# pypr/pysph

Hardware: AMD Instinct MI355X
Metric: particle-updates/sec (nnps.update + AccelerationEval.compute), WCSPH 3D, fp64 (higher is better)
Workload: dtype f64

## Files before the change

pysph_amd/csrc/sph_eval.hip:

```cpp
#include "sph_internal.h"
#include "sph_kernels.h"
#include "sph_pair.h"

#include <cfloat>
#include <cmath>
#include <type_traits>

#ifndef SPH_KERNEL_UNIT
#define SPH_KERNEL_UNIT 0
#endif
#define SPH_PRIMARY_UNIT (SPH_KERNEL_UNIT == 0)

#if SPH_PRIMARY_UNIT

struct EosArgs {
    int kind;
    double par[SPH_MAX_PAR];
    double *rho, *p, *cs;
    size_t start, stop;
    double *q[SPH_PROP_COUNT];
    uint32_t *tflag;
};

__device__ inline void jacobi_eigen3(double A[3][3], double V[3][3], double d[3])
// ... 304 lines not shown
#pragma unroll
            for (int q = 0; q < MAX_AUX / 2; q++) pc[2 + q] = make_double2(v[2 * q], v[2 * q + 1]);
            np = a.nr / 2;
        }
        emit_pieces(a, i, pc, np);
    } else {
        a.posh[a.off + i] = ph;
        double *dst = a.aux + (a.off + i) * (size_t)a.na;
#pragma unroll
        for (int k = 0; k < MAX_AUX; k++) if (k < a.na) dst[k] = v[k];
    }
}

struct PackMArgs {
    const uint32_t *perm;
    const uint8_t *slot;
    size_t n, off;
    const double *prop[9][SPH_MAX_ARRAYS];
    int vh;
    uint32_t cls;
    double *rec;
    float4 *fpos;
    int f32, lds_np;
    double gmin[3];
    double hr;
    uint32_t *rho_flag;
};

template <bool F32, bool VH>
__global__ __launch_bounds__(256) void k_pack_merged(PackMArgs a)
{
    const size_t i = (size_t)blockIdx.x * blockDim.x + threadIdx.x;
    if (i >= a.n) return;
    const uint32_t o = a.perm[i], sl = a.slot[i];
    double v[8];
#pragma unroll
    for (int k = 0; k < 8; k++) {
        const double *p = kernarg_read<const double *>(__builtin_offsetof(PackMArgs, prop) + ((size_t)k * SPH_MAX_ARRAYS + sl) * sizeof(double *));
        v[k] = p[o];
    }
    const double rho = v[6];
    const double q = rho != 0.0 ? v[7] * (1.0 / (rho * rho)) : 0.0;
    const double srho = ((a.cls >> sl) & 1u) ? -rho : rho;
    if (!(rho > 0.0) && fabs(v[0]) < SPH_PARKED_MIN) atomicOr(a.rho_flag, 1u);
    double hp = 0.0;
    if (VH) hp = kernarg_read<const double *>(__builtin_offsetof(PackMArgs, prop) + ((size_t)8 * SPH_MAX_ARRAYS + sl) * sizeof(double *))[o];
    a.fpos[i] = make_float4((float)(v[0] - a.gmin[0]), (float)(v[1] - a.gmin[1]), (float)(v[2] - a.gmin[2]),
                            VH ? (float)(a.hr * hp) : (float)a.hr);
    double2 pc[PACK_MAXP];
#pragma unroll
    for (int k = 0; k < PACK_MAXP; k++) pc[k] = make_double2(0.0, 0.0);
    int np;
    if (VH && F32) {
        pc[0] = __builtin_bit_cast(double2, make_float4((float)(v[0] - a.gmin[0]), (float)(v[1] - a.gmin[1]), (float)(v[2] - a.gmin[2]), (float)hp));
        pc[1] = __builtin_bit_cast(double2, make_float4((float)v[3], (float)v[4], (float)v[5], (float)srho));
        np = 2;
    } else if (VH) {
        pc[0] = make_double2(v[0], v[1]); pc[1] = make_double2(v[2], hp);
        pc[2] = make_double2(v[3], v[4]); pc[3] = make_double2(v[5], srho);
        np = 4;
    } else if (F32) {
        pc[0] = __builtin_bit_cast(double2, make_float4((float)(v[0] - a.gmin[0]), (float)(v[1] - a.gmin[1]), (float)(v[2] - a.gmin[2]), (float)v[3]));
        pc[1] = __builtin_bit_cast(double2, make_float4((float)v[4], (float)v[5], (float)srho, (float)q));
        np = 2;
    } else {
        pc[0] = make_double2(v[0], v[1]); pc[1] = make_double2(v[2], v[3]);
        pc[2] = make_double2(v[4], v[5]); pc[3] = make_double2(srho, q);
        np = 4;
    }
    emit_pieces(a, i, pc, np);
}

template <class T> struct FamWCSPH_T {
    typedef T Real;
    static constexpr uint32_t CF0 = F_CONT | F_MOM | F_XSPH;
#ifndef SPH_WCSPH_MINB
#define SPH_WCSPH_MINB 4
#endif
    static constexpr int MINB = SPH_WCSPH_MINB;
    static constexpr int NA = 8;
    static constexpr int NR = 12;
    struct Params {
        T c0, alpha, beta, gx, gy, gz, eps;
        double *arho, *au, *av, *aw, *ax, *ay, *az, *dt_cfl, *dt_force;
    };
    struct Dest {
        T u, v, w, rho, p, cs, tmpi;
        T arho, au, av, aw, ax, ay, az, dt_cfl;
    };
    template <class A> static __device__ __forceinline__ void load(Dest &D, const T *a, const A &, uint32_t)
    {
        D.u = a[0]; D.v = a[1]; D.w = a[2]; D.rho = a[4]; D.tmpi = a[5]; D.cs = a[6]; D.p = a[7];
        D.arho = D.au = D.av = D.aw = D.ax = D.ay = D.az = T(0.0);
        D.dt_cfl = T(-1.0);
    }
    static constexpr bool PRED = true;
    template <int KK, bool UH, class A>
    static __device__ __forceinline__ void pair(Dest &D, const real4<T> &pi, const real4<T> &pj, T r2,
                                                const T (&s)[NA], uint32_t fl, const A &a, bool pass = true)
    {
        PairGeomT<T> g;
        constexpr bool MRG = SPH_MERGED_RSQ && sizeof(T) == 8 && !SphKernel<KK>::CUTOFF;
        T tt_m = T(0.0);
        if constexpr (MRG) {
            if (fl & F_MOM) tt_m = pair_geom_mom<KK, UH>(g, pi, pj, r2, T(0.5) * (D.rho + s[4]), a);
            else pair_geom<KK, UH>(g, pi, pj, r2, a);
        } else {
            pair_geom<KK, UH>(g, pi, pj, r2, a);
        }
        const T tg = pair_gradfac<KK, UH>(g);
        const T vij0 = D.u - s[0], vij1 = D.v - s[1], vij2 = D.w - s[2];
        const T vdotx = vij0 * g.xij[0] + vij1 * g.xij[1] + vij2 * g.xij[2];
        const T mj = pass ? s[3] : T(0.0);
        if (fl & F_CONT) D.arho = fma(mj * tg, vdotx, D.arho);
        if (fl & (F_MOM | F_XSPH)) {
            const T rhoij = T(0.5) * (D.rho + s[4]);
            T rhoij1;
            T wij = T(0.0);
            if (fl & (F_XSPH | F_TENSILE)) wij = pair_w<KK, UH>(g);
            if (fl & F_MOM) {
                const T re = r2 + g.eps;
                const T tt = MRG ? tt_m : fast_rcp(re * rhoij);
                const T inv_re = rhoij * tt;
                rhoij1 = re * tt;
                const T hv = g.hij * vdotx;
                const T muij = raw_min(hv, T(0.0)) * inv_re;
                const T cij = T(0.5) * (D.cs + s[6]);
                const T piij = (a.p.beta * muij - a.p.alpha * cij) * muij * rhoij1;
                const T dtv = fabs(hv * (g.rinv * g.rinv));
                D.dt_cfl = raw_max(D.dt_cfl, (r2 > T(1e-12) && pass) ? dtv : T(-1.0));
                const T tmpj = s[5];
                T tmp = D.tmpi + tmpj;
                if (fl & F_TENSILE) {
                    const T qd = (a.k.deltap * g.hij) * g.h1;
                    const T wdp = SphKernel<KK>::w(qd, g.dim) * g.fac;
                    T fij = wij * fast_rcp(wdp);
                    fij = fij * fij;
                    fij = fij * fij;
                    const T Ri = D.p > 0 ? T(0.01) * D.tmpi : T(0.2) * fabs(D.tmpi);
                    const T Rj = s[7] > 0 ? T(0.01) * tmpj : T(0.2) * fabs(tmpj);
                    tmp = (D.tmpi + tmpj) + (Ri + Rj) * fij;
                }
                const T ft = -mj * (tmp + piij) * tg;
                D.au = fma(ft, g.xij[0], D.au);
                D.av = fma(ft, g.xij[1], D.av);
                D.aw = fma(ft, g.xij[2], D.aw);
            } else {
                rhoij1 = fast_rcp(rhoij);
            }
            if (fl & F_XSPH) {
                const T tmp = -a.p.eps * mj * wij * rhoij1;
                D.ax = fma(tmp, vij0, D.ax);
                D.ay = fma(tmp, vij1, D.ay);
                D.az = fma(tmp, vij2, D.az);
            }
        }
    }
    template <class A> static __device__ __forceinline__ void finish(Dest &D, const A &a, uint32_t o)
    {
        if (a.dflags & F_CONT) a.p.arho[o] = D.arho;
        if (a.dflags & F_MOM) {
            T au = D.au + a.p.gx, av = D.av + a.p.gy, aw = D.aw + a.p.gz;
            a.p.au[o] = au; a.p.av[o] = av; a.p.aw[o] = aw;
            a.p.dt_cfl[o] = D.dt_cfl < T(0.0) ? T(0.0) : D.dt_cfl + a.p.c0;
            a.p.dt_force[o] = au * au + av * av + aw * aw;
        }
        if (a.dflags & F_XSPH) {
            a.p.ax[o] = D.ax + D.u; a.p.ay[o] = D.ay + D.v; a.p.az[o] = D.az + D.w;
        }
    }
};
typedef FamWCSPH_T<double> FamWCSPH;

template <class T, bool UM = false> struct FamWCSPHE_T : FamWCSPH_T<T> {
    static constexpr bool EOSF = true;
    static constexpr bool UMASS = UM;
    static constexpr int NR = 8;
    struct Raw {
        typename std::conditional<sizeof(T) == 8, double2, float4>::type q[sizeof(T) == 8 ? 4 : 2];
    };
    template <class A> static __device__ __forceinline__ void load_raw(const A &a, uint32_t jg, Raw &r)
    {
        if constexpr (sizeof(T) == 8) {
            const double2 *p = reinterpret_cast<const double2 *>(a.rec) + (unsigned long long)jg * 4;
            r.q[0] = p[0]; r.q[1] = p[1]; r.q[2] = p[2]; r.q[3] = p[3];
        } else {
            const float4 *p = reinterpret_cast<const float4 *>(a.rec) + (unsigned long long)jg * 2;
            r.q[0] = p[0]; r.q[1] = p[1];
        }
    }
    template <class A> static __device__ __forceinline__ void decode(const A &a, const Raw &r, uint32_t fl, T mu, real4<T> &pj, T (&s)[8],
                                                                     int gk = 3)
    {
        T rho;
        if constexpr (sizeof(T) == 8) {
            pj.x = r.q[0].x; pj.y = r.q[0].y; pj.z = r.q[1].x; pj.w = 0.0;
            s[0] = r.q[1].y; s[1] = r.q[2].x; s[2] = r.q[2].y; s[3] = r.q[3].y; rho = r.q[3].x;
        } else {
            pj.x = r.q[0].x; pj.y = r.q[0].y; pj.z = r.q[0].z; pj.w = 0.f;
            s[0] = r.q[0].w; s[1] = r.q[1].x; s[2] = r.q[1].y; s[3] = r.q[1].w; rho = r.q[1].z;
        }
        s[4] = rho;
        s[5] = s[6] = s[7] = T(0.0);
        if constexpr (UM) {
            const T q = s[3];
            s[3] = mu;
            if (fl & F_MOM) {
                const T ratio = rho * (T)a.e_rho01;
                s[5] = q;
                s[6] = (T)a.e_c0 * tait_cs_power(ratio, gk);
            }
        } else
        if (fl & F_MOM) {
            const T ratio = rho * (T)a.e_rho01;
            T r7, r3;
            tait_powers(ratio, gk, r7, r3);
            const T p = (T)a.e_p0 + (T)a.e_B * (r7 - T(1.0));
            s[5] = rho != T(0.0) ? p * fast_rcp(rho * rho) : T(0.0);
            s[6] = (T)a.e_c0 * r3;
            s[7] = p;
        }
    }
    template <class A> static __device__ __forceinline__ void load_fused(const A &a, uint32_t jg, uint32_t fl, T mu, real4<T> &pj, T (&s)[8])
    {
        Raw r;
        load_raw(a, jg, r);
        decode(a, r, fl, mu, pj, s);
    }
};

template <class T, bool UM = false> struct FamWCSPHEG_T : FamWCSPHE_T<T, UM> {
    typedef FamWCSPHE_T<T, UM> Base;
    template <class A> static __device__ __forceinline__ void load_fused(const A &a, uint32_t jg, uint32_t fl, T mu, real4<T> &pj, T (&s)[8])
    {
        typename Base::Raw r;
        Base::load_raw(a, jg, r);
        Base::decode(a, r, fl, mu, pj, s, a.e_gk);
    }
};

template <class T> struct FamWCSPHV_T : FamWCSPH_T<T> {
    static constexpr bool EOSF = true;
    static constexpr int NR = 8;
    template <class A> static __device__ __forceinline__ void load_fused(const A &a, uint32_t jg, uint32_t fl, T mu, real4<T> &pj, T (&s)[8])
    {
        T rho;
        if constexpr (sizeof(T) == 8) {
            const double2 *p = reinterpret_cast<const double2 *>(a.rec) + (unsigned long long)jg * 4;
            const double2 q0 = p[0], q1 = p[1], q2 = p[2], q3 = p[3];
            pj.x = q0.x; pj.y = q0.y; pj.z = q1.x; pj.w = q1.y;
            s[0] = q2.x; s[1] = q2.y; s[2] = q3.x; rho = q3.y;
        } else {
            const float4 *p = reinterpret_cast<const float4 *>(a.rec) + (unsigned long long)jg * 2;
            const float4 q0 = p[0], q1 = p[1];
            pj.x = q0.x; pj.y = q0.y; pj.z = q0.z; pj.w = q0.w;
            s[0] = q1.x; s[1] = q1.y; s[2] = q1.z; rho = q1.w;
        }
        s[3] = mu;
        s[4] = rho;
        s[5] = s[6] = s[7] = T(0.0);
        if (fl & F_MOM) {
            const T ratio = rho * (T)a.e_rho01;
            T r7, r3;
            tait_powers(ratio, 3, r7, r3);
            const T p = (T)a.e_p0 + (T)a.e_B * (r7 - T(1.0));
            s[5] = rho != T(0.0) ? p * fast_rcp(rho * rho) : T(0.0);
            s[6] = (T)a.e_c0 * r3;
            s[7] = p;
        }
    }
};

#define WCSPHM_CT(f00, f01, f10, f11) ((uint32_t)(f00) | ((uint32_t)(f01) << 4) | ((uint32_t)(f10) << 8) | ((uint32_t)(f11) << 12))
template <class T> struct FamWCSPHM_T : FamWCSPHE_T<T, true> {
    typedef FamWCSPHE_T<T, true> Base;
    typedef typename Base::Raw Raw;
    static constexpr bool MERGED = true;
    static constexpr uint32_t CF0 = WCSPHM_CT(F_CONT | F_MOM | F_XSPH, F_CONT | F_MOM, F_CONT, 0);
    struct Params {
        T c0, alpha, beta, gx, gy, gz, eps;
        double mu1;
        uint32_t rng[SPH_MAX_ARRAYS][2];
        double *out[SPH_MAX_ARRAYS][9];
    };
    static __device__ __forceinline__ size_t rng_offset(uint32_t slot) { return __builtin_offsetof(Params, rng) + (size_t)slot * 8; }
    struct Dest : Base::Dest { bool dc; };
    template <class A> static __device__ __forceinline__ void load(Dest &D, const T *a, const A &A_, uint32_t o, uint32_t)
    {
        Base::load(D, a, A_, o);
        D.dc = a[3] < T(0.0);
    }
    template <class A> static __device__ __forceinline__ void decode(const A &a, const Raw &r, uint32_t, T mu, real4<T> &pj, T (&s)[8])
    {
        T rho, q;
        if constexpr (sizeof(T) == 8) {
            pj.x = r.q[0].x; pj.y = r.q[0].y; pj.z = r.q[1].x; pj.w = 0.0;
            s[0] = r.q[1].y; s[1] = r.q[2].x; s[2] = r.q[2].y; q = r.q[3].y; rho = r.q[3].x;
        } else {
            pj.x = r.q[0].x; pj.y = r.q[0].y; pj.z = r.q[0].z; pj.w = 0.f;
            s[0] = r.q[0].w; s[1] = r.q[1].x; s[2] = r.q[1].y; q = r.q[1].w; rho = r.q[1].z;
        }
        const bool c1 = rho < T(0.0);
        s[3] = c1 ? -(T)a.p.mu1 : mu;
        rho = fabs(rho);
        s[4] = rho;
        const T ratio = rho * (T)a.e_rho01;
        s[5] = q;
        s[6] = (T)a.e_c0 * tait_cs_power(ratio, 3);
        s[7] = T(0.0);
    }
    template <class A> static __device__ __forceinline__ void load_fused(const A &a, uint32_t jg, uint32_t fl, T mu, real4<T> &pj, T (&s)[8])
    {
        Raw r;
        Base::load_raw(a, jg, r);
        decode(a, r, fl, mu, pj, s);
    }
    static __device__ __forceinline__ bool acts(uint32_t ct, uint32_t bit, bool dc, bool sc)
    {
        const bool c00 = ct & bit, c01 = (ct >> 4) & bit, c10 = (ct >> 8) & bit, c11 = (ct >> 12) & bit;
        return dc ? (sc ? c11 : c10) : (sc ? c01 : c00);
    }
    template <int KK, bool UH, class A>
    static __device__ __forceinline__ void pair(Dest &D, const real4<T> &pi, const real4<T> &pj, T r2,
                                                const T (&s)[8], uint32_t ct, const A &a, bool pass = true)
    {
        PairGeomT<T> g;
        constexpr bool MRG = SPH_MERGED_RSQ && sizeof(T) == 8 && !SphKernel<KK>::CUTOFF;
        T tt_m = T(0.0);
        if constexpr (MRG) tt_m = pair_geom_mom<KK, UH>(g, pi, pj, r2, T(0.5) * (D.rho + s[4]), a);
        else pair_geom<KK, UH>(g, pi, pj, r2, a);
        const T tg = pair_gradfac<KK, UH>(g);
        const T vij0 = D.u - s[0], vij1 = D.v - s[1], vij2 = D.w - s[2];
        const T vdotx = vij0 * g.xij[0] + vij1 * g.xij[1] + vij2 * g.xij[2];
        const bool sc = s[3] < T(0.0);
        const T m = fabs(s[3]);
        const bool on_c = pass && acts(ct, F_CONT, D.dc, sc), on_m = pass && acts(ct, F_MOM, D.dc, sc),
                   on_x = pass && acts(ct, F_XSPH, D.dc, sc);
        D.arho = fma((on_c ? m : T(0.0)) * tg, vdotx, D.arho);
        const T rhoij = T(0.5) * (D.rho + s[4]);
        const T wij = pair_w<KK, UH>(g);
        const T re = r2 + g.eps;
        const T tt = MRG ? tt_m : fast_rcp(re * rhoij);
        const T inv_re = rhoij * tt;
        const T rhoij1 = re * tt;
        const T hv = g.hij * vdotx;
        const T muij = raw_min(hv, T(0.0)) * inv_re;
        const T cij = T(0.5) * (D.cs + s[6]);
        const T piij = (a.p.beta * muij - a.p.alpha * cij) * muij * rhoij1;
        const T dtv = fabs(hv * (g.rinv * g.rinv));
        D.dt_cfl = raw_max(D.dt_cfl, (r2 > T(1e-12) && on_m) ? dtv : T(-1.0));
        const T ft = -(on_m ? m : T(0.0)) * ((D.tmpi + s[5]) + piij) * tg;
        D.au = fma(ft, g.xij[0], D.au);
        D.av = fma(ft, g.xij[1], D.av);
        D.aw = fma(ft, g.xij[2], D.aw);
        const T tmp = -a.p.eps * (on_x ? m : T(0.0)) * wij * rhoij1;
        D.ax = fma(tmp, vij0, D.ax);
        D.ay = fma(tmp, vij1, D.ay);
        D.az = fma(tmp, vij2, D.az);
    }
    template <class A> static __device__ __forceinline__ void finish(Dest &D, const A &a, uint32_t o, uint32_t slot)
// ... 1342 lines not shown
                for (auto &pc : c->pack_cache)
                    if (pc.epoch == c->pack_epoch && (pc.fam != fam || pc.sig != sig)) keep = false;
            if (!keep)
                for (auto &pc : c->pack_cache) pc.epoch = 0;
            auto pack_once = [&](int id, size_t off, uint32_t fl, bool dest_only) -> int {
                PackCache &pc = c->pack_cache[id];
                const bool hit = share && pc.epoch == c->pack_epoch && pc.fam == fam && pc.sig == sig;
                if (phase != 2 || repack) SPH_TRY(pack_array(c, id, off, pl, fam, fl, dest_only, !hit, 0));
                if (phase != 1 && c->arr[id].g_n > 0) SPH_TRY(pack_array(c, id, off, pl, fam, fl, dest_only, !hit, 1));
                pc.epoch = share ? c->pack_epoch : 0; pc.fam = fam; pc.sig = sig;
                return SPH_OK;
            };
            for (int j = 0; j < nsrcs; j++) SPH_TRY(pack_once(srcs[j], off_of[j], srcs[j] == dst ? dflags : sflags[j], false));
            if (!dest_is_src) SPH_TRY(pack_once(dst, d_off, dflags, true));
        }

        int nl_mode = 0;
        if (c->nl_reuse && !c->row_lds && c->pair_variant == 6 && nsrcs == 1 && g->nl_mode && !c->ablate && !any_ghosts && phase == 0) {
            const size_t n_wt = (size_t)4 * div_up(D.n, 256);
            if (g->nl_mode == 1) {
                SPH_TRY(c->nlbuf.reserve(n_wt * NLW * sizeof(uint32_t)));
                c->nl.valid = true; c->nl.epoch = c->nnps_epoch; c->nl.dst = dst; c->nl.src = srcs[0];
                c->nl.start = start; c->nl.stop = stop; c->nl.nd = D.n;
                nl_mode = 1;
            } else if (g->nl_mode == 2 && c->nl.valid && c->nl.epoch == c->nnps_epoch && c->nl.dst == dst && c->nl.src == srcs[0] &&
                       c->nl.nd == D.n && c->nl.start <= start && c->nl.stop >= stop && c->nlbuf.bytes >= n_wt * NLW * sizeof(uint32_t)) {
                nl_mode = 2;
            }
        } else if (g->nl_mode != 2) {
            c->nl.valid = c->nl.valid && !(g->nl_mode == 1);
        }

        if (phase == 1 && !c->split_pair) continue;
        ScopedTimer tm(c, T_PAIR);
        ScopedTimer tmf(c, T_PAIR_FAM + fam);
        if (phase == 2) c->timers[T_N_PHASE2].count++;
        if (eosf || tvff || eosv) c->timers[T_N_EOSF].count++;
        if (umass || tvff || elu || eosv) c->timers[T_N_UMASS].count++;
        if (nl_mode == 1) c->timers[T_N_NLKEEP].count++;
        if (nl_mode == 2) c->timers[T_N_NLREUSE].count++;
        {
            int nseg = nsrcs;
            for (int j = 0; j < nsrcs; j++) nseg += c->arr[srcs[j]].g_n > 0 && phase != 1;
            if (nseg > SPH_MAX_ARRAYS) { sph_set_error("too many source segments (%d arrays with ghost segments)", nsrcs); return SPH_ERR_UNSUPPORTED; }
        }
        auto common = [&](auto &a) {
            fill_common(c, a, K, t);
            a.nsrc = 0;
            for (int j = 0; j < nsrcs; j++) {
                const DevArray &S = c->arr[srcs[j]];
                a.src[a.nsrc++] = {S.cell_start.as<uint32_t>(), (uint32_t)off_of[j], sflags[j], S.fine_start.as<uint32_t>(), S.m_value, 0u};
            }
            for (int j = 0; j < nsrcs && phase != 1; j++) {
                const DevArray &S = c->arr[srcs[j]];
                if (S.g_n == 0) continue;
                a.src[a.nsrc++] = {S.g_cell_start.as<uint32_t>(), (uint32_t)(off_of[j] + S.n_binned), sflags[j],
                                   S.g_fine_start.as<uint32_t>(), S.m_value, 1u};
            }
            a.face_mode = c->split_pair ? phase : 0;
            a.d_off = (uint32_t)d_off; a.nd = (uint32_t)D.n_binned;
            a.d_mu = D.m_value;
            a.d_keys = D.keys_sorted.as<uint32_t>(); a.d_fkeys = D.fkeys_sorted.as<uint32_t>(); a.d_perm = D.perm.as<uint32_t>();
            set_tile_order(c, a, D);
            a.d_start = (uint32_t)start; a.d_stop = (uint32_t)stop; a.dflags = dflags;
            a.nl = nullptr; a.nl_mode = nl_mode;
            if (nl_mode) a.nl = c->nlbuf.as<uint32_t>();
            if (start == 0 && stop == D.n_real && D.n_binned == D.n && !any_ghosts) use_dest_list(c, a, D);
            if (eosf || eosv) {
                a.e_rho01 = 1.0 / g->eos_par[0]; a.e_c0 = g->eos_par[1];
                a.e_B = g->eos_par[0] * g->eos_par[1] * g->eos_par[1] / g->eos_par[2];
        a.e_gk = tait_gk(g->eos_par[2]);
                a.e_p0 = g->eos_par[3];
            }
            if (tvff) { a.e_p0 = g->eos_par[0]; a.e_rho01 = 1.0 / g->eos_par[1]; a.e_B = g->eos_par[2]; }
        };
        auto run_wcsph = [&](auto tag) -> int {
            typedef decltype(tag) F;
            PairArgs<F> a;
            memset(&a, 0, sizeof a);
            common(a);
            const sph_equation *me = eq_of[SPH_EQ_MOMENTUM], *xe = eq_of[SPH_EQ_XSPH];
            if (me) { a.p.c0 = me->par[0]; a.p.alpha = me->par[1]; a.p.beta = me->par[2]; a.p.gx = me->par[3]; a.p.gy = me->par[4]; a.p.gz = me->par[5]; }
            if (xe) a.p.eps = xe->par[0];
            if (dflags & F_CONT) { SPH_TRY(ensure_out(c, dst, {SPH_ARHO})); a.p.arho = D.prop[SPH_ARHO]; }
            if (dflags & F_MOM) {
                SPH_TRY(ensure_out(c, dst, {SPH_AU, SPH_AV, SPH_AW, SPH_DT_CFL, SPH_DT_FORCE}));
                a.p.au = D.prop[SPH_AU]; a.p.av = D.prop[SPH_AV]; a.p.aw = D.prop[SPH_AW];
                a.p.dt_cfl = D.prop[SPH_DT_CFL]; a.p.dt_force = D.prop[SPH_DT_FORCE];
            }
            if (dflags & F_XSPH) {
                SPH_TRY(ensure_out(c, dst, {SPH_AX, SPH_AY, SPH_AZ}));
                a.p.ax = D.prop[SPH_AX]; a.p.ay = D.prop[SPH_AY]; a.p.az = D.prop[SPH_AZ];
            }
            if constexpr (std::is_same<F, FamWCSPHV_T<typename F::Real>>::value) return launch_pair_fused<F, false>(c, K->kind, a);
            else if constexpr (fam_eosf<F>::value) return launch_pair_fused<F>(c, K->kind, a);
            else return launch_pair<F>(c, K->kind, a);
        };
        auto run_density = [&](auto tag) -> int {
            typedef decltype(tag) F;
            PairArgs<F> a;
            memset(&a, 0, sizeof a);
            common(a);
            SPH_TRY(ensure_out(c, dst, {SPH_RHO}));
            a.p.rho = D.prop[SPH_RHO];
            if (dflags & F_TVFSD) { SPH_TRY(ensure_out(c, dst, {SPH_VOL})); a.p.V = D.prop[SPH_VOL]; }
            if ((dflags & F_SD) && (dflags & F_TVFSD)) { sph_set_error("both SummationDensity flavours on one destination"); return SPH_ERR_UNSUPPORTED; }
            return launch_pair<F>(c, K->kind, a);
        };
        auto run_vgrad = [&](auto tag) -> int {
            typedef decltype(tag) F;
            PairArgs<F> a;
            memset(&a, 0, sizeof a);
            common(a);
            static const int vp[9] = {SPH_V00, SPH_V01, SPH_V02, SPH_V10, SPH_V11, SPH_V12, SPH_V20, SPH_V21, SPH_V22};
            if ((dflags & F_VG2) && (dflags & F_VG3)) { sph_set_error("both VelocityGradient2D and 3D on one destination"); return SPH_ERR_UNSUPPORTED; }
            for (int k = 0; k < 9; k++) {
                const bool used = (dflags & F_VG3) || (k == 0 || k == 1 || k == 3 || k == 4);
                if (used) { SPH_TRY(sph_array_ensure_prop(c, dst, vp[k])); a.p.v[k] = D.prop[vp[k]]; }
            }
            return launch_pair<F>(c, K->kind, a);
        };
        auto run_elastic = [&](auto tag) -> int {
            typedef decltype(tag) F;
            PairArgs<F> a;
            memset(&a, 0, sizeof a);
            common(a);
            const sph_equation *se = eq_of[SPH_EQ_MOMENTUM_WITH_STRESS], *ae = eq_of[SPH_EQ_MONAGHAN_ART_VISCOSITY],
                               *xe = eq_of[SPH_EQ_XSPH];
            if (se) { a.p.wdeltap = se->par[0]; a.p.n = se->par[1]; }
            a.p.tension = nullptr;
            if (elu && c->tension_flag && nsrcs == 1 && c->arr[srcs[0]].tflag_valid && c->arr[srcs[0]].tflag.ptr) {
                a.p.tension = c->arr[srcs[0]].tflag.as<uint32_t>();
                c->timers[T_N_TFLAG].count++;
            }
            if (ae) { a.p.alpha = ae->par[0]; a.p.beta = ae->par[1]; }
            if (xe) a.p.eps = xe->par[0];
            if (dflags & F_ECONT) { SPH_TRY(ensure_out(c, dst, {SPH_ARHO})); a.p.arho = D.prop[SPH_ARHO]; }
            if (dflags & (F_ESTRESS | F_EAV)) {
                SPH_TRY(ensure_out(c, dst, {SPH_AU, SPH_AV, SPH_AW}));
                a.p.au = D.prop[SPH_AU]; a.p.av = D.prop[SPH_AV]; a.p.aw = D.prop[SPH_AW];
            }
            if (dflags & F_EXSPH) {
                SPH_TRY(ensure_out(c, dst, {SPH_AX, SPH_AY, SPH_AZ}));
                a.p.ax = D.prop[SPH_AX]; a.p.ay = D.prop[SPH_AY]; a.p.az = D.prop[SPH_AZ];
            }
            if constexpr (fam_eosf<F>::value) return launch_pair_fused<F>(c, K->kind, a);
            else return launch_pair<F>(c, K->kind, a);
        };
        auto run_tvf = [&](auto tag) -> int {
            typedef decltype(tag) F;
            PairArgs<F> a;
            memset(&a, 0, sizeof a);
            common(a);
            const sph_equation *pe = eq_of[SPH_EQ_TVF_MOM_PRESSURE], *ve = eq_of[SPH_EQ_TVF_MOM_VISCOSITY],
                               *ae = eq_of[SPH_EQ_TVF_MOM_ART_VISCOSITY];
            if (pe) { a.p.pb = pe->par[0]; a.p.gx = pe->par[1]; a.p.gy = pe->par[2]; a.p.gz = pe->par[3]; a.p.tdamp = pe->par[4]; }
            if (ve) a.p.nu = ve->par[0];
            if (ae) { a.p.c0 = ae->par[0]; a.p.alpha = ae->par[1]; }
            SPH_TRY(ensure_out(c, dst, {SPH_AU, SPH_AV, SPH_AW}));
            a.p.au = D.prop[SPH_AU]; a.p.av = D.prop[SPH_AV]; a.p.aw = D.prop[SPH_AW];
            a.p.m = D.prop[SPH_M];
            if (dflags & F_TP) {
                SPH_TRY(ensure_out(c, dst, {SPH_AUHAT, SPH_AVHAT, SPH_AWHAT}));
                a.p.auhat = D.prop[SPH_AUHAT]; a.p.avhat = D.prop[SPH_AVHAT]; a.p.awhat = D.prop[SPH_AWHAT];
            }
            if constexpr (fam_eosf<F>::value) return launch_pair_fused<F>(c, K->kind, a);
// ... 358 lines not shown
```

pysph_amd/csrc/sph_pair.h:

```cpp
#pragma once

#include <hip/hip_runtime.h>
#include <cstdint>

#include "sphhip.h"
#include "sph_kernels.h"

template <class T> __device__ __forceinline__ T r2_exact(T dx, T dy, T dz)
{
#pragma clang fp contract(off)
    const T a = dx * dx, b = dy * dy, c = dz * dz;
    return (a + b) + c;
}

template <class T> struct Real4Of;
template <> struct Real4Of<double> { typedef double4 type; };
template <> struct Real4Of<float> { typedef float4 type; };
template <class T> using real4 = typename Real4Of<T>::type;


struct KernelConst {
    double sigma;
    double deltap;
    int dim;
};


struct SrcDesc {
    const uint32_t *cell_start;
    uint32_t off;
    uint32_t flags;
    const uint32_t *fine_start;
    double mu;
    uint32_t ghost;
};

static __host__ __device__ inline int tait_gk(double gamma)
{
    return gamma == 7.0 ? 3 : gamma == 5.0 ? 2 : gamma == 3.0 ? 1 : gamma == 1.0 ? 0 : -1;
}
template <class T> __device__ __forceinline__ T tait_cs_power(T ratio, int gk)
{
    if (gk == 3) return (ratio * ratio) * ratio;
    if (gk == 2) return ratio * ratio;
    return gk == 1 ? ratio : T(1.0);
}
template <class T> __device__ __forceinline__ void tait_powers(T ratio, int gk, T &rg, T &rk)
{
    const T r2 = ratio * ratio;
    if (gk == 3) { rk = r2 * ratio; rg = (r2 * r2) * rk; }
    else if (gk == 2) { rk = r2; rg = (r2 * r2) * ratio; }
    else if (gk == 1) { rk = ratio; rg = r2 * ratio; }
    else { rk = T(1.0); rg = ratio; }
}

template <class Fam> struct PairArgs {
    int nsrc;
    SrcDesc src[SPH_MAX_ARRAYS];
    const double4 *posh;
    const double *aux;
    const double *rec;
    int nrec;
    const float4 *fpos;
    double dom_extent;
    uint32_t d_off, nd;
    double d_mu;
    const uint32_t *d_keys, *d_fkeys, *d_perm;
    const uint8_t *d_slot;
    const uint32_t *d_tile_order;
    const uint32_t *d_list;
    int face_mode, gfx_lo, gfx_hi;
    int row_mod3;
    uint32_t d_start, d_stop;
    int nc[3];
    double xmin[3];
    double cell_size;
    double radius_scale;
    KernelConst k;
    uint32_t dflags;
    unsigned long long *dbg;
    int ablate;
    int skip_init;
    int skip_post;
    double t, dt;
    double hu, h1u, facu, epsu, hr2u;
    uint32_t *nl;
    int nl_mode;
    int norm_masks;
    double e_rho01, e_c0, e_B, e_p0;
    int e_gk;
    typename Fam::Params p;
};

template <class F, class = void> struct fam_merged { static constexpr bool value = false; };
template <class F> struct fam_merged<F, decltype((void)F::MERGED)> { static constexpr bool value = F::MERGED; };

template <class V> __device__ __forceinline__ V kernarg_read(size_t byte_offset)
{
    typedef const char __attribute__((address_space(4))) *kptr;
    const kptr ka = (kptr)__builtin_amdgcn_kernarg_segment_ptr();
    return *reinterpret_cast<const V __attribute__((address_space(4))) *>(ka + byte_offset);
}

template <class F, class = void> struct fam_token { static constexpr bool value = false; };
template <class F> struct fam_token<F, decltype((void)F::TOKEN)> { static constexpr bool value = F::TOKEN; };

template <class F, class = void> struct fam_eosf { static constexpr bool value = false; };
template <class F> struct fam_eosf<F, decltype((void)F::EOSF)> { static constexpr bool value = F::EOSF; };

template <class F, class = void> struct fam_pair_index { static constexpr bool value = false; };
template <class F> struct fam_pair_index<F, decltype((void)F::PAIR_INDEX)> { static constexpr bool value = F::PAIR_INDEX; };


#ifndef SPH_NEWTON_STEPS
#define SPH_NEWTON_STEPS 1
#endif
__device__ __forceinline__ double fast_rcp(double d)
{
    double x = __builtin_amdgcn_rcp(d);
    double e = fma(-d, x, 1.0);
    x = fma(x, e, x);
    if (SPH_NEWTON_STEPS > 1) {
        e = fma(-d, x, 1.0);
        x = fma(x, e, x);
    }
    return x;
}
__device__ __forceinline__ void fast_sqrt_rsqrt(double a, double &s, double &rs)
{
    a = raw_max(a, 1e-300);
    double y = __builtin_amdgcn_rsq(a);
    double g = a * y, h = 0.5 * y;
    double r = fma(-h, g, 0.5);
    g = fma(g, r, g);
    h = fma(h, r, h);
    if (SPH_NEWTON_STEPS > 1) {
        r = fma(-h, g, 0.5);
        g = fma(g, r, g);
        h = fma(h, r, h);
    }
    s = g;
    rs = h + h;
}
__device__ __forceinline__ float fast_rcp(float d) { return __builtin_amdgcn_rcpf(d); }
__device__ __forceinline__ void fast_sqrt_rsqrt(float a, float &s, float &rs)
{
    a = fmaxf(a, 1e-35f);
    rs = __builtin_amdgcn_rsqf(a);
    s = a * rs;
}

template <class T> struct PairGeomT {
    T xij[3];
    T r2, rij, rinv, hij, h1, q, fac, eps;
    int dim;
};
typedef PairGeomT<double> PairGeom;

template <int KK, bool UH, class T, class A>
__device__ __forceinline__ void pair_geom(PairGeomT<T> &g, const real4<T> &pi, const real4<T> &pj, T r2, const A &a)
{
    g.xij[0] = pi.x - pj.x; g.xij[1] = pi.y - pj.y; g.xij[2] = pi.z - pj.z;
    g.r2 = r2;
    constexpr bool EXACT_Q = SphKernel<KK>::CUTOFF;
    if (EXACT_Q) {
        g.rij = sqrt(r2);
        g.rinv = g.rij > T(0) ? T(1) / g.rij : T(0);
    } else {
        fast_sqrt_rsqrt(r2, g.rij, g.rinv);
    }
    if (UH) {
        g.hij = (T)a.hu; g.h1 = (T)a.h1u; g.fac = (T)a.facu; g.eps = (T)a.epsu;
    } else {
        g.hij = T(0.5) * (pi.w + pj.w);
        g.h1 = EXACT_Q ? T(1) / g.hij : fast_rcp(g.hij);
        g.fac = kernel_norm((T)a.k.sigma, g.h1, a.k.dim);
        g.eps = T(0.01) * g.hij * g.hij;
    }
    g.q = g.rij * g.h1;
    g.dim = a.k.dim;
}
#ifndef SPH_MERGED_RSQ
#define SPH_MERGED_RSQ 0
#endif
template <int KK, bool UH, class A>
__device__ __forceinline__ double pair_geom_mom(PairGeomT<double> &g, const double4 &pi, const double4 &pj, double r2, double rhoij, const A &a)
{
    typedef double T;
    g.xij[0] = pi.x - pj.x; g.xij[1] = pi.y - pj.y; g.xij[2] = pi.z - pj.z;
    g.r2 = r2;
    if (UH) {
        g.hij = (T)a.hu; g.h1 = (T)a.h1u; g.fac = (T)a.facu; g.eps = (T)a.epsu;
    } else {
        g.hij = T(0.5) * (pi.w + pj.w);
        g.h1 = fast_rcp(g.hij);
        g.fac = kernel_norm((T)a.k.sigma, g.h1, a.k.dim);
        g.eps = T(0.01) * g.hij * g.hij;
    }
    const T P = (r2 + g.eps) * rhoij;
    const T r2c = raw_max(r2, 1e-300);
    const T aa = r2c * (P * P);
    const T y = __builtin_amdgcn_rsq(aa);
    T gg = aa * y, hh = 0.5 * y;
    const T rr = fma(-hh, gg, 0.5);
    hh = fma(hh, rr, hh);
    const T t = hh + hh;
    g.rinv = t * P;
    g.rij = r2c * g.rinv;
    g.q = g.rij * g.h1;
    g.dim = a.k.dim;
    return t * g.rij;
}

template <int KK, bool UH, class T> __device__ __forceinline__ T pair_w(const PairGeomT<T> &g) { return SphKernel<KK>::template w<UH>(g.q, g.dim) * g.fac; }
template <int KK, bool UH, class T> __device__ __forceinline__ T pair_gradh(const PairGeomT<T> &g, int dim)
{
    const T v = g.fac * g.h1 * (SphKernel<KK>::template dw<UH>(g.q, dim) * g.q + SphKernel<KK>::template w<UH>(g.q, dim) * (T)dim);
    return SphKernel<KK>::GRADH_FLIPPED ? v : -v;
}
template <int KK, bool UH, class T> __device__ __forceinline__ T pair_gradfac(const PairGeomT<T> &g)
{
    T t;
    if (SphKernel<KK>::HAS_DWQ) t = SphKernel<KK>::template dwq<UH>(g.q, g.dim) * (g.fac * g.h1 * g.h1);
    else t = SphKernel<KK>::template dw<UH>(g.q, g.dim) * (g.fac * g.h1) * g.rinv;
    return g.rij > T(1e-12) ? t : T(0);
}

__device__ __forceinline__ float prefilter_slack(const float4 &fp, float slack, float dom_extent)
{
    const float am = fmaxf(fmaxf(fabsf(fp.x), fabsf(fp.y)), fabsf(fp.z));
    return am > dom_extent ? fmaxf(slack, am * 3.0e-6f) : slack;
}
// ... 93 lines not shown

    const int t = threadIdx.x & 63;
    const uint32_t wt = xcd_tile(blockIdx.x, gridDim.x) * WPB + (uint32_t)wv;
    uint32_t dtile = wt >> 2;
    if (dtile * 256u >= a.nd) return;
    if (a.d_tile_order) dtile = a.d_tile_order[dtile];
    const uint32_t tbase = dtile * 256u + (wt & 3u) * 64u;
    const uint32_t i = tbase + t;
    if (tbase >= a.nd) return;
    const bool valid = i < a.nd;
    uint32_t ic = valid ? i : a.nd - 1;
    if (a.d_list) ic = a.d_list[ic];
    const uint32_t o = a.d_perm[ic];
    uint32_t slot = 0;
    bool active;
    if constexpr (fam_merged<Fam>::value) {
        slot = a.d_slot[ic];
        const unsigned long long rg = kernarg_read<unsigned long long>(__builtin_offsetof(PairArgs<Fam>, p) + Fam::rng_offset(slot));
        active = valid && o >= (uint32_t)rg && o < (uint32_t)(rg >> 32);
    } else {
        active = valid && o >= a.d_start && o < a.d_stop;
    }
    const uint32_t fkey = a.d_fkeys[ic];
    const uint32_t key = fkey / SPH_NSUB;
    const int ncx = a.nc[0], ncy = a.nc[1], ncz = a.nc[2];
    const int row = key / ncx;
    const int cx = (int)(key % ncx) * SPH_NSUB + (int)(fkey % SPH_NSUB);
    bool facew = true;
    if (a.face_mode != 0 || a.gfx_lo > -0x7fffffff || a.gfx_hi < 0x7fffffff) {
        int mn = active ? cx : 0x7fffffff, mx = active ? cx : -0x7fffffff;
#pragma unroll
        for (int o = 32; o > 0; o >>= 1) { mn = min(mn, __shfl_xor(mn, o, 64)); mx = max(mx, __shfl_xor(mx, o, 64)); }
        mn = __builtin_amdgcn_readfirstlane(mn); mx = __builtin_amdgcn_readfirstlane(mx);
        facew = mn <= mx && (mn - XWIN <= a.gfx_lo || mx + XWIN >= a.gfx_hi);
        if (mn > mx && !a.nl_mode) return;
        if (a.face_mode == 1 && facew) return;
        if (a.face_mode == 2 && !facew) return;
    }
    real4<T> pi;
    typename Fam::Dest D;
    uint32_t wtok = 0;
    if constexpr (fam_token<Fam>::value) wtok = Fam::wave_token(a);
    T cur_mu = (T)a.d_mu;
    auto fetch = [&](uint32_t jg, uint32_t flags, real4<T> &pj, T (&sj)[Fam::NA]) {
        if constexpr (fam_token<Fam>::value) Fam::load_fused(a, jg, flags, cur_mu, pj, sj, wtok);
        else if constexpr (fam_eosf<Fam>::value) Fam::load_fused(a, jg, flags, cur_mu, pj, sj);
        else if constexpr (F32) load_record_f32<Fam, T>(reinterpret_cast<const float *>(a.rec) + (unsigned long long)jg * NR, pj, sj);
        else load_record<Fam, UH>(a.rec + (unsigned long long)jg * NR, flags, pj, sj);
    };
    {
        T sd_[Fam::NA];
        fetch(a.d_off + ic, a.dflags, pi, sd_);
        if (UH) pi.w = (T)a.hu;
        if constexpr (fam_merged<Fam>::value) Fam::load(D, sd_, a, o, slot);
        else Fam::load(D, sd_, a, o);
    }
    const int nfx = ncx * SPH_NSUB;
    const T hi_r = (T)a.radius_scale * pi.w;
    const T hi2 = UH ? (T)a.hr2u : hi_r * hi_r;
    const int row_first = __builtin_amdgcn_readfirstlane(row), row_last = __builtin_amdgcn_readlane(row, 63);
    if (DBGC(a) && t == 0) atomicAdd(DBGC(a) + 2, 1ull);

    auto do_pair = [&](uint32_t jg, uint32_t flags) {
        real4<T> pj;
        T sj[Fam::NA];
        fetch(jg, flags, pj, sj);
        pin_record<Fam::NA, T>(pj, sj);
        T hj2 = hi2;
        if (!UH) { hj2 = (T)a.radius_scale * pj.w; hj2 *= hj2; }
        const T r2 = r2_exact<T>(pi.x - pj.x, pi.y - pj.y, pi.z - pj.z);
        if (((r2 < hi2) || (r2 < hj2)) && ABLATE(a) != 1) {
            if constexpr (fam_pair_index<Fam>::value) Fam::template pair<KK, UH>(D, pi, pj, r2, sj, flags, a, jg);
            else Fam::template pair<KK, UH>(D, pi, pj, r2, sj, flags, a);
        }
    };

    int cq = 0;
    auto phase2 = [&](uint32_t flags) {
        unsigned long long m = 0;
        uint32_t jb = 0;
        int q = 0;
        if (cq > 0 && ABLATE(a) != 2) { m = smask[0][t]; jb = sjb[0][t]; }
        const uint32_t self = a.d_off + ic;
        if (__any(m != 0)) {
            if (DBGC(a) && t == 0) atomicAdd(DBGC(a) + 1, 1ull);
            do {
                if (DBGC(a) && t == 0) atomicAdd(DBGC(a), 1ull);
                const bool has = m != 0;
                uint32_t j = has ? jb + (uint32_t)__builtin_ctzll(m) : self;
                m &= m - 1;
                if (m == 0 && q + 1 < cq) { ++q; m = smask[q][t]; jb = sjb[q][t]; }
                if (ABLATE(a) == 3) j = self;
                if constexpr (Fam::PRED) {
                    real4<T> pj;
                    T sj[Fam::NA];
                    fetch(j, flags, pj, sj);
                    T hj2 = hi2;
                    if (!UH) { hj2 = (T)a.radius_scale * pj.w; hj2 *= hj2; }
                    const T r2 = r2_exact<T>(pi.x - pj.x, pi.y - pj.y, pi.z - pj.z);
                    const bool pass = has && ((r2 < hi2) || (r2 < hj2)) && ABLATE(a) != 1;
                    Fam::template pair<KK, UH>(D, pi, pj, r2, sj, flags, a, pass);
                } else {
                    if (has) do_pair(j, flags);
                }
            } while (__any(m != 0));
        }
        cq = 0;
    };

    uint32_t *const nlw = a.nl_mode ? a.nl + (size_t)wt * NLW : nullptr;
    bool reuse = false, unsaved = false;
    if (a.nl_mode == 2) {
        const uint32_t nq = nlw[t];
        reuse = !__any(nq == NL_NONE);
        if (reuse) {
            const uint32_t off0 = a.src[0].off;
            const int nqmax = wave_max_i32((int)nq);
            for (int q = 0; q < nqmax; q++) {
                const uint32_t *w = nlw + 64 * (1 + 3 * q) + t;
                smask[q][t] = (unsigned long long)w[0] | ((unsigned long long)w[64] << 32);
                sjb[q][t] = w[128] + off0;
            }
            __builtin_amdgcn_fence(__ATOMIC_ACQ_REL, "wavefront");
            cq = active ? (int)nq : 0;
        }
    }

    for (int s = 0; s < a.nsrc; s++) {
    const SrcDesc sd = a.src[s];
    if (sd.ghost && !facew) continue;
    const uint32_t fl = CF ? CF : sd.flags;
    cur_mu = (T)sd.mu;
    int R = row_first, st = 0, part_resume = 0;
    uint32_t tb_resume = 0;
    bool resumed = false;
    for (;;) {
    bool more = false;
    for (; R <= row_last && !more && !reuse && ABLATE(a) != 6; R++, st = 0) {
        const bool inseg = active && row == R;
        const unsigned long long segm = __ballot(inseg);
        if (!segm) continue;
        const int cxa = __builtin_amdgcn_readlane(cx, __builtin_ctzll(segm));
        const int cxb = __builtin_amdgcn_readlane(cx, 63 - __builtin_clzll(segm));
        const int cyR = R % ncy, czR = R / ncy;
        const int xa = max(cxa - XWIN, 0), xb = min(cxb + XWIN, nfx - 1);
        const int ncs = xb - xa + 2;
        const double binw = a.cell_size * (1.0 / SPH_NSUB);
        const float oxf = (float)(binw * xa);
        const float oyf = (float)(a.cell_size * (cyR - 1));
        const float ozf = (float)(a.cell_size * (czR - 1));
        const double L = fmax(a.cell_size * (double)max((xb - xa) / SPH_NSUB + 2, 4), a.dom_extent);
        const float slack = (float)(L * 1.5e-6);
        const float4 fpi = a.fpos[a.d_off + ic];
        const float fxs = fpi.x - oxf, fys = fpi.y - oyf, fzs = fpi.z - ozf;
        const f2 fx = {fxs, fxs}, fy = {fys, fys}, fz = {fzs, fzs};
        const float hif = (float)hi_r * 1.000001f + prefilter_slack(fpi, slack, (float)a.dom_extent);
        const float hi2f = hif * hif;
        const int mycl = max(cx - XWIN, xa) - xa, mych = min(cx + XWIN, xb) + 1 - xa;

        for (; st < 9; st++) {
            const int st2 = a.row_mod3 == 4 ? (st + (int)(wt % 9u)) % 9 : st;
            const int sy = st2 % 3 - 1, sz = st2 / 3 - 1;
            const int dy = (a.row_mod3 & 1) ? (sy + 1 - cyR % 3 + 4) % 3 - 1 : sy;
            const int dz = (a.row_mod3 & 2) ? (sz + 1 - czR % 3 + 4) % 3 - 1 : sz;
            const int yy = cyR + dy, zz = czR + dz;
            if (yy < 0 || yy >= ncy || zz < 0 || zz >= ncz) continue;
            const uint32_t rowb = (uint32_t)(ncx * (yy + ncy * zz)) * SPH_NSUB;
            const uint32_t j0 = sd.fine_start[rowb + xa], j1 = sd.fine_start[rowb + xb + 1];
            const bool csl_ok = ncs <= WCSL && j1 - j0 < 65536u;
            uint32_t tb = j0;
            int part = 0;
            if (resumed) { tb = tb_resume; part = part_resume; resumed = false; }
            const bool csl_now = tb != j0;
            for (; tb < j1; tb += WCAP, part = 0) {
                const int tn = (int)min((uint32_t)WCAP, j1 - tb);
                if (DBGC(a) && t == 0) atomicAdd(DBGC(a) + 3, 1ull);
                if (csl_ok && (tb == j0 || csl_now))
                    for (int q = t; q < ncs; q += 64) csl[q] = (unsigned short)(sd.fine_start[rowb + xa + q] - j0);
                for (int k = t; k < tn + 8; k += 64) {
                    float vx = 3.0e18f, vy = 3.0e18f, vz = 3.0e18f, vw = 0.f;
                    if (k < tn) {
                        const float4 fj = a.fpos[sd.off + tb + k];
                        vx = fj.x - oxf; vy = fj.y - oyf; vz = fj.z - ozf;
                        const float hjf = fj.w * 1.000001f + (UH ? slack : prefilter_slack(fj, slack, (float)a.dom_extent));
                        vw = hjf * hjf;
                    }
                    tx[k] = vx; ty[k] = vy; tz[k] = vz;
                    if (!UH) tw[k] = vw;
// ... 272 lines not shown
```

Before: 1.930 billion.

## Fold WCSPH pair constants and pin loop registers in the neighbor loop

Folds the 0.5 factors of rho_ij and c_ij into pre-doubled beta and eps parameters, which are cached in per-destination registers. Inline asm barriers pin these values, plus the neighbor index and queue counter, into VGPRs for the Wendland quintic loop, so they are not rematerialised or turned into scalar loads. Also trims one FMA from the sqrt/rsqrt Newton step, selects only the upper word for the dt_cfl mask, and restructures the mask-advance loop condition. The extra live registers may lower occupancy, and the upper-word select relies on the low bits of dtv matching those of -1.0 being harmless.

Result: no change. 1.948 billion, median of 6 (+0.9%).

```diff
diff --git a/pysph_amd/csrc/sph_eval.hip b/pysph_amd/csrc/sph_eval.hip
--- a/pysph_amd/csrc/sph_eval.hip
+++ b/pysph_amd/csrc/sph_eval.hip
@@ -410,15 +410,25 @@
     static constexpr int NR = 12;
     struct Params {
         T c0, alpha, beta, gx, gy, gz, eps;
+        T beta2, eps2;
         double *arho, *au, *av, *aw, *ax, *ay, *az, *dt_cfl, *dt_force;
     };
     struct Dest {
         T u, v, w, rho, p, cs, tmpi;
         T arho, au, av, aw, ax, ay, az, dt_cfl;
+        T alpha, beta2, eps2;
     };
-    template <class A> static __device__ __forceinline__ void load(Dest &D, const T *a, const A &, uint32_t)
+    static constexpr bool LOOP_REGS = true;
+    template <int KK> static __device__ __forceinline__ void loop_regs(Dest &D, T &)
+    {
+        if constexpr (KK == SPH_K_WENDLAND_QUINTIC) asm volatile("" : "+v"(D.alpha), "+v"(D.beta2), "+v"(D.eps2));
+    }
+    template <class A> static __device__ __forceinline__ void load(Dest &D, const T *a, const A &args, uint32_t)
     {
         D.u = a[0]; D.v = a[1]; D.w = a[2]; D.rho = a[4]; D.tmpi = a[5]; D.cs = a[6]; D.p = a[7];
+        if constexpr (std::is_same<typename std::decay<decltype(args.p)>::type, Params>::value) {
+            D.alpha = args.p.alpha; D.beta2 = args.p.beta2; D.eps2 = args.p.eps2;
+        }
         D.arho = D.au = D.av = D.aw = D.ax = D.ay = D.az = T(0.0);
         D.dt_cfl = T(-1.0);
     }
@@ -431,7 +441,7 @@
         constexpr bool MRG = SPH_MERGED_RSQ && sizeof(T) == 8 && !SphKernel<KK>::CUTOFF;
         T tt_m = T(0.0);
         if constexpr (MRG) {
-            if (fl & F_MOM) tt_m = pair_geom_mom<KK, UH>(g, pi, pj, r2, T(0.5) * (D.rho + s[4]), a);
+            if (fl & F_MOM) tt_m = pair_geom_mom<KK, UH>(g, pi, pj, r2, D.rho + s[4], a);
             else pair_geom<KK, UH>(g, pi, pj, r2, a);
         } else {
             pair_geom<KK, UH>(g, pi, pj, r2, a);
@@ -442,21 +452,21 @@
         const T mj = pass ? s[3] : T(0.0);
         if (fl & F_CONT) D.arho = fma(mj * tg, vdotx, D.arho);
         if (fl & (F_MOM | F_XSPH)) {
-            const T rhoij = T(0.5) * (D.rho + s[4]);
-            T rhoij1;
+            const T rho2 = D.rho + s[4];
+            T rhoij1h;
             T wij = T(0.0);
             if (fl & (F_XSPH | F_TENSILE)) wij = pair_w<KK, UH>(g);
             if (fl & F_MOM) {
                 const T re = r2 + g.eps;
-                const T tt = MRG ? tt_m : fast_rcp(re * rhoij);
-                const T inv_re = rhoij * tt;
-                rhoij1 = re * tt;
+                const T tt = MRG ? tt_m : fast_rcp(re * rho2);
+                const T inv_re = rho2 * tt;
+                rhoij1h = re * tt;
                 const T hv = g.hij * vdotx;
                 const T muij = raw_min(hv, T(0.0)) * inv_re;
-                const T cij = T(0.5) * (D.cs + s[6]);
-                const T piij = (a.p.beta * muij - a.p.alpha * cij) * muij * rhoij1;
-                const T dtv = fabs(hv * (g.rinv * g.rinv));
-                D.dt_cfl = raw_max(D.dt_cfl, (r2 > T(1e-12) && pass) ? dtv : T(-1.0));
+                const T c2 = D.cs + s[6];
+                const T piij = (D.beta2 * muij - D.alpha * c2) * muij * rhoij1h;
+                const T dtv = fabs(hv) * (g.rinv * g.rinv);
+                D.dt_cfl = raw_max(D.dt_cfl, upper_word_or<T>(r2 > T(1e-12) && pass, dtv, T(-1.0)));
                 const T tmpj = s[5];
                 T tmp = D.tmpi + tmpj;
                 if (fl & F_TENSILE) {
@@ -474,10 +484,10 @@
                 D.av = fma(ft, g.xij[1], D.av);
                 D.aw = fma(ft, g.xij[2], D.aw);
             } else {
-                rhoij1 = fast_rcp(rhoij);
+                rhoij1h = fast_rcp(rho2);
             }
             if (fl & F_XSPH) {
-                const T tmp = -a.p.eps * mj * wij * rhoij1;
+                const T tmp = -D.eps2 * mj * wij * rhoij1h;
                 D.ax = fma(tmp, vij0, D.ax);
                 D.ay = fma(tmp, vij1, D.ay);
                 D.az = fma(tmp, vij2, D.az);
@@ -504,6 +514,11 @@
     static constexpr bool EOSF = true;
     static constexpr bool UMASS = UM;
     static constexpr int NR = 8;
+    template <int KK> static __device__ __forceinline__ void loop_regs(typename FamWCSPH_T<T>::Dest &D, T &mu)
+    {
+        FamWCSPH_T<T>::template loop_regs<KK>(D, mu);
+        if constexpr (UM && KK == SPH_K_WENDLAND_QUINTIC) asm volatile("" : "+v"(mu));
+    }
     struct Raw {
         typename std::conditional<sizeof(T) == 8, double2, float4>::type q[sizeof(T) == 8 ? 4 : 2];
     };
@@ -604,6 +619,10 @@
     typedef FamWCSPHE_T<T, true> Base;
     typedef typename Base::Raw Raw;
     static constexpr bool MERGED = true;
+    template <int KK> static __device__ __forceinline__ void loop_regs(typename Base::Dest &, T &mu)
+    {
+        if constexpr (KK == SPH_K_WENDLAND_QUINTIC) asm volatile("" : "+v"(mu));
+    }
     static constexpr uint32_t CF0 = WCSPHM_CT(F_CONT | F_MOM | F_XSPH, F_CONT | F_MOM, F_CONT, 0);
     struct Params {
         T c0, alpha, beta, gx, gy, gz, eps;
@@ -2112,6 +2131,7 @@
             const sph_equation *me = eq_of[SPH_EQ_MOMENTUM], *xe = eq_of[SPH_EQ_XSPH];
             if (me) { a.p.c0 = me->par[0]; a.p.alpha = me->par[1]; a.p.beta = me->par[2]; a.p.gx = me->par[3]; a.p.gy = me->par[4]; a.p.gz = me->par[5]; }
             if (xe) a.p.eps = xe->par[0];
+            a.p.beta2 = a.p.beta + a.p.beta; a.p.eps2 = a.p.eps + a.p.eps;
             if (dflags & F_CONT) { SPH_TRY(ensure_out(c, dst, {SPH_ARHO})); a.p.arho = D.prop[SPH_ARHO]; }
             if (dflags & F_MOM) {
                 SPH_TRY(ensure_out(c, dst, {SPH_AU, SPH_AV, SPH_AW, SPH_DT_CFL, SPH_DT_FORCE}));
diff --git a/pysph_amd/csrc/sph_pair.h b/pysph_amd/csrc/sph_pair.h
--- a/pysph_amd/csrc/sph_pair.h
+++ b/pysph_amd/csrc/sph_pair.h
@@ -105,6 +105,9 @@
 template <class F, class = void> struct fam_token { static constexpr bool value = false; };
 template <class F> struct fam_token<F, decltype((void)F::TOKEN)> { static constexpr bool value = F::TOKEN; };
 
+template <class F, class = void> struct fam_loop_regs { static constexpr bool value = false; };
+template <class F> struct fam_loop_regs<F, decltype((void)F::LOOP_REGS)> { static constexpr bool value = F::LOOP_REGS; };
+
 template <class F, class = void> struct fam_eosf { static constexpr bool value = false; };
 template <class F> struct fam_eosf<F, decltype((void)F::EOSF)> { static constexpr bool value = F::EOSF; };
 
@@ -133,14 +136,14 @@
     double g = a * y, h = 0.5 * y;
     double r = fma(-h, g, 0.5);
     g = fma(g, r, g);
-    h = fma(h, r, h);
     if (SPH_NEWTON_STEPS > 1) {
+        h = fma(h, r, h);
         r = fma(-h, g, 0.5);
         g = fma(g, r, g);
-        h = fma(h, r, h);
+        y = h + h;
     }
     s = g;
-    rs = h + h;
+    rs = fma(y, r, y);
 }
 __device__ __forceinline__ float fast_rcp(float d) { return __builtin_amdgcn_rcpf(d); }
 __device__ __forceinline__ void fast_sqrt_rsqrt(float a, float &s, float &rs)
@@ -148,6 +151,17 @@
     a = fmaxf(a, 1e-35f);
     rs = __builtin_amdgcn_rsqf(a);
     s = a * rs;
+}
+
+template <class T> __device__ __forceinline__ T upper_word_or(bool c, T x, T y)
+{
+    if constexpr (sizeof(T) == 8) {
+        const unsigned long long xb = __builtin_bit_cast(unsigned long long, x), yb = __builtin_bit_cast(unsigned long long, y);
+        const uint32_t hi = c ? (uint32_t)(xb >> 32) : (uint32_t)(yb >> 32);
+        return __builtin_bit_cast(double, ((unsigned long long)hi << 32) | (uint32_t)xb);
+    } else {
+        return c ? x : y;
+    }
 }
 
 template <class T> struct PairGeomT {
@@ -407,14 +421,22 @@
         int q = 0;
         if (cq > 0 && ABLATE(a) != 2) { m = smask[0][t]; jb = sjb[0][t]; }
         const uint32_t self = a.d_off + ic;
-        if (__any(m != 0)) {
+        bool left = m != 0;
+        if (__any(left)) {
             if (DBGC(a) && t == 0) atomicAdd(DBGC(a) + 1, 1ull);
+            if constexpr (UH && fam_loop_regs<Fam>::value) Fam::template loop_regs<KK>(D, cur_mu);
             do {
                 if (DBGC(a) && t == 0) atomicAdd(DBGC(a), 1ull);
-                const bool has = m != 0;
+                const bool has = left;
                 uint32_t j = has ? jb + (uint32_t)__builtin_ctzll(m) : self;
+                asm volatile("" : "+v"(j));
                 m &= m - 1;
-                if (m == 0 && q + 1 < cq) { ++q; m = smask[q][t]; jb = sjb[q][t]; }
+                if (m == 0) {
+                    ++q;
+                    asm volatile("" : "+v"(q));
+                    if (q < cq) { m = smask[q][t]; jb = sjb[q][t]; }
+                }
+                left = m != 0;
                 if (ABLATE(a) == 3) j = self;
                 if constexpr (Fam::PRED) {
                     real4<T> pj;
@@ -428,7 +450,7 @@
                 } else {
                     if (has) do_pair(j, flags);
                 }
-            } while (__any(m != 0));
+            } while (__any(left));
         }
         cq = 0;
     };
```
